# mvenouziou/Boosted_DETR

Measured on AMD Instinct MI355X. Metric: images/sec training step (fwd+matcher+loss+bwd), 640x640 N=100, higher is better.
Workload: dtype f32 (conv/GEMM products as 3 split-f16 [fwd] / split-bf16 [grad] MFMA products, f32 accumulate)

## Files before the change

boosted_detr_amd/_lib.py:

```python
from __future__ import annotations

import ctypes as C
import os
from pathlib import Path

_LIB_PATH = Path(os.environ.get("BDETR_LIB") or Path(__file__).resolve().parent / "csrc" / "libbdetr.so")
_lib = None

c_f32p = C.c_void_p
c_i32p = C.c_void_p
c_i64p = C.c_void_p
c_stream = C.c_void_p


class ConvDesc(C.Structure):
    _fields_ = [(n, C.c_int) for n in ("N", "H", "W", "C", "K", "R", "S", "stride", "pad", "OH", "OW")]


class GemmDesc(C.Structure):
    _fields_ = [
        ("I", C.c_int), ("J", C.c_int), ("R", C.c_int), ("nb0", C.c_int), ("nb1", C.c_int),
        ("a", C.c_void_p), ("lda", C.c_int64), ("sa0", C.c_int64), ("sa1", C.c_int64), ("a_rcontig", C.c_int),
        ("b", C.c_void_p), ("ldb", C.c_int64), ("sb0", C.c_int64), ("sb1", C.c_int64), ("b_rcontig", C.c_int),
        ("c", C.c_void_p), ("ldc", C.c_int64), ("sc0", C.c_int64), ("sc1", C.c_int64),
        ("bias", C.c_void_p), ("alpha", C.c_float), ("act", C.c_int), ("accumulate", C.c_int), ("splitk", C.c_int),
        ("grad", C.c_int),
    ]


class BnAffine(C.Structure):
    _fields_ = [("mean", C.c_void_p), ("rstd", C.c_void_p), ("gamma", C.c_void_p), ("beta", C.c_void_p)]


class BnBwdFuse(C.Structure):
    _fields_ = [("y", C.c_void_p), ("mean", C.c_void_p), ("rstd", C.c_void_p), ("gamma", C.c_void_p), ("beta", C.c_void_p), ("relu", C.c_int),
                ("part_g", C.c_void_p), ("part_gx", C.c_void_p), ("relu_mask", C.c_void_p),
                ("y2", C.c_void_p), ("mean2", C.c_void_p), ("rstd2", C.c_void_p), ("part_gx2", C.c_void_p)]


class RowchainFwdDesc(C.Structure):
    _fields_ = ([("M", C.c_int64), ("nstages", C.c_int), ("eps", C.c_float), ("rate", C.c_float), ("ctx", C.c_void_p), ("resid", C.c_void_p),
                 ("w", C.c_void_p * 3), ("bias", C.c_void_p * 3)]
                + [(n, C.c_void_p) for n in ("g1", "b1", "g2", "b2", "pre1", "x1", "mean1", "rstd1", "h", "pre2", "x2", "mean2", "rstd2")]
                + [("seed1", C.c_uint64), ("seed2", C.c_uint64), ("seed_base", C.c_void_p)])


class RowchainBwdDesc(C.Structure):
    _fields_ = ([("M", C.c_int64), ("nstages", C.c_int), ("rate", C.c_float)]
                + [(n, C.c_void_p) for n in ("dout", "pre2", "mean2", "rstd2", "g2", "h", "pre1", "mean1", "rstd1", "g1")]
                + [("wt", C.c_void_p * 3)]
                + [(n, C.c_void_p) for n in ("G2", "G1", "G0", "dresid", "dctx", "partials")]
                + [("seed1", C.c_uint64), ("seed2", C.c_uint64), ("seed_base", C.c_void_p)])
# ... 27 lines not shown
    "bdetr_prof_dump": (I, [C.c_char_p]),
    "bdetr_image_prep": (I, [P, I, I, I, P, I, I, P]),
    "bdetr_tokens_prepare": (I, [P, P, L, I, I, I, P, P, P]),
    "bdetr_augment_ws_floats": (I, [I]),
    "bdetr_augment": (I, [P, P, P, P, I, I, I, P, P]),
    "bdetr_jpeg_quality_ws_bytes": (C.c_int64, [I, I, I]),
    "bdetr_jpeg_quality": (I, [P, P, P, I, I, I, P, P]),
    "bdetr_augment_jpeg": (I, [P, P, P, P, P, I, I, I, P, P, P]),
    "bdetr_conv2d_fwd": (I, [P, P, P, P, C.POINTER(ConvDesc), I, P, P, P]),
    "bdetr_conv2d_fwd_stat_chunks": (I, [C.POINTER(ConvDesc)]),
    "bdetr_conv2d_bwd_data": (I, [P, P, P, C.POINTER(ConvDesc), I, P]),
    "bdetr_conv2d_bwd_weight": (I, [P, P, P, C.POINTER(ConvDesc), I, P]),
    "bdetr_conv2d_bwd_weight_splitk": (I, [C.POINTER(ConvDesc)]),
    "bdetr_bn_apply_p16": (I, [P, P, P, P, P, P, I, C.POINTER(BnAffine), I, P, P, P, P, P, L, I, P]),
    "bdetr_bn_bwd_p16": (I, [P, P, I, P, P, P, P, P, I, I, P, P, P, P, P, P, P, P, I, L, I, P]),
    "bdetr_bn_bwd_p16_even_pixels": (I, [P, P, I, P, P, P, P, P, I, I, P, P, P, P, P, P, I, I, I, I, I, P]),
    "bdetr_p16_supported": (I, [C.POINTER(ConvDesc)]),
    "bdetr_p16_pack": (I, [P, L, P, P, P, P]),
    "bdetr_p16_unpack": (I, [P, I, L, P, P]),
    "bdetr_p16_pack_conv_weights": (I, [P, I, I, I, I, P, P, P, P]),
    "bdetr_p16_pack_conv_weights_multi": (I, [P, I, P, P]),
    "bdetr_p16_conv2d_fwd_stat_chunks": (I, [C.POINTER(ConvDesc)]),
    "bdetr_p16_conv2d_fwd": (I, [P, P, P, P, C.POINTER(ConvDesc), I, P, P, P]),
    "bdetr_p16_conv2d_bwd_data": (I, [P, P, P, C.POINTER(ConvDesc), I, P]),
    "bdetr_p16_conv2d_bwd_data_stat_chunks": (I, [C.POINTER(ConvDesc)]),
    "bdetr_p16_conv2d_bwd_data_masked_accum": (I, [P, P, P, P, C.POINTER(ConvDesc), C.POINTER(BnBwdFuse), P]),
    "bdetr_p16_conv2d_bwd_data_masked_accum_compact": (I, [P, P, P, P, P, C.POINTER(ConvDesc), C.POINTER(BnBwdFuse), P]),
    "bdetr_relu_mask_apply": (I, [P, P, C.c_int64, P]),
    "bdetr_p16_conv2d_bwd_data_bnstats": (I, [P, P, P, C.POINTER(ConvDesc), C.POINTER(BnBwdFuse), P]),
    "bdetr_p16_conv2d_bwd_weight_splitk": (I, [C.POINTER(ConvDesc)]),
    "bdetr_p16_conv2d_bwd_weight": (I, [P, P, P, C.POINTER(ConvDesc), I, P]),
    "bdetr_p16_conv2d_bwd_weight_xf16": (I, [P, P, P, C.POINTER(ConvDesc), I, P]),
    "bdetr_gemm": (I, [C.POINTER(GemmDesc), P]),
    "bdetr_gemm_ws": (I, [C.POINTER(GemmDesc), P, L, P]),
    "bdetr_splitk_workspace_elems": (L, [L, L, I]),
    "bdetr_conv2d_bwd_weight_ws": (I, [P, P, P, C.POINTER(ConvDesc), I, P, L, P]),
    "bdetr_p16_conv2d_bwd_weight_ws": (I, [P, I, P, P, C.POINTER(ConvDesc), I, P, L, P]),
    "bdetr_gemm_grouped": (I, [C.POINTER(GemmDesc), I, P]),
    "bdetr_colsum_chunks": (I, [L]),
    "bdetr_colsum": (I, [P, L, I, P, P, P]),
# ... 107 lines not shown
```

boosted_detr_amd/csrc/gemm_common.h:

```cpp
#pragma once
#include "common.h"
#include <type_traits>

namespace bdgemm {

enum { ST_STORE = 0, ST_ACCUM = 1, ST_ATOMIC = 2 };
enum { AR_FP32 = 0, AR_BF16X3 = 1, AR_FP16X3 = 2, AR_P16_F16 = 3, AR_P16_BF16 = 4, AR_BF16X6 = 5 };

struct GemmParams {
    int I, J, R;
    int nb1;
    int splitk, r_chunk;
    int tiles_i, tiles_j;
    float* c; int64_t ldc, sc0, sc1;
    const float* bias; float alpha; int act; int mode;
    float* stat_sum; float* stat_sq;
    int vec_store;
    int rowmap;
    int rm_OW, rm_OHOW, rm_H, rm_W, rm_stride;
    int rm_off;
    int ngroups;
    const float* ga[4]; const float* gb[4]; float* gc[4]; const float* gbias[4]; int gI[4];
    const float* bnb_y; const float* bnb_mean; const float* bnb_rstd; const float* bnb_gamma; const float* bnb_beta;
    int bnb_relu; float* bnb_sum_g; float* bnb_sum_gx;
    const unsigned long long* bnb_mask;
    const float* bnb2_y; const float* bnb2_mean; const float* bnb2_rstd; float* bnb2_sum_gx;
    const unsigned long long* acc_mask;
    const float* acc_src; int acc_H, acc_W;
    int b_f16;
#ifdef BDETR_SGEMM_DIAG
    int dbg;
#endif
};

#ifdef BDETR_SGEMM_DIAG
#define BDETR_DBG(g, bits) (((g).dbg & (bits)) != 0)
#else
#define BDETR_DBG(g, bits) false
#endif

inline void init_params(GemmParams& g) {
// ... 174 lines not shown
                            if constexpr (MASKED) on = ((bbits[k] >> e) & 1u) != 0u;
                            else on = !g.bnb_relu || (__builtin_fmaf(yv[k][e] - bnv[0][e], bnv[1][e] * bnv[2][e], bnv[3][e]) > 0.f);
                            const float ge = on ? val[k][e] : 0.f;
                            bnv[4][e] += ge; bnv[5][e] += ge * ((yv[k][e] - bnv[0][e]) * bnv[1][e]);
                            if constexpr (BNB2) bn2[2][e] += ge * ((y2v[k][e] - bn2[0][e]) * bn2[1][e]);
                        }
                    }
                }
            }
            if constexpr (BNB) {
                static_assert(NT * 8 <= LDS_FLOATS, "reduction scratch must fit");
                __syncthreads();
                *reinterpret_cast<f32x4*>(lds + tid * 8) = bnv[4];
                *reinterpret_cast<f32x4*>(lds + tid * 8 + 4) = bnv[5];
                __syncthreads();
                if (tid < V_PER_ROW && jok) {
                    f32x4 a = {0, 0, 0, 0}, b = a;
#pragma unroll
                    for (int k = 0; k < RSTEP; ++k) {
                        a += *reinterpret_cast<const f32x4*>(lds + (tid + k * V_PER_ROW) * 8);
                        b += *reinterpret_cast<const f32x4*>(lds + (tid + k * V_PER_ROW) * 8 + 4);
                    }
                    *reinterpret_cast<f32x4*>(g.bnb_sum_g + (int64_t)tile_i * g.J + jc) = a;
                    *reinterpret_cast<f32x4*>(g.bnb_sum_gx + (int64_t)tile_i * g.J + jc) = b;
                }
                if constexpr (BNB2) {
                    __syncthreads();
                    *reinterpret_cast<f32x4*>(lds + tid * 4) = bn2[2];
                    __syncthreads();
                    if (tid < V_PER_ROW && jok) {
                        f32x4 c = {0, 0, 0, 0};
#pragma unroll
                        for (int k = 0; k < RSTEP; ++k) c += *reinterpret_cast<const f32x4*>(lds + (tid + k * V_PER_ROW) * 4);
                        *reinterpret_cast<f32x4*>(g.bnb2_sum_gx + (int64_t)tile_i * g.J + jc) = c;
                    }
                }
            }
        };
        using T = std::true_type; using F = std::false_type;
        const bool accum = g.mode == ST_ACCUM;
        if constexpr (BNB2_ONLY) { vec_out(F{}, T{}, T{}, T{}, T{}, F{}); return; }
        if constexpr (COMPACT_ONLY) {
            if (g.bnb_y != nullptr) vec_out(F{}, T{}, T{}, T{}, F{}, T{});
            else vec_out(F{}, T{}, F{}, T{}, F{}, T{});
            return;
// ... 59 lines not shown
```

boosted_detr_amd/csrc/norm.hip:

```cpp
#include "common.h"
#include "p16.h"

namespace {

struct ColGeom { int tx, ty, gx; };
inline ColGeom col_geom(int C) {
    int c4 = C / 4;
    int tx = 1; while (tx < c4 && tx < 64) tx <<= 1;
    ColGeom g; g.tx = tx; g.ty = 256 / tx; g.gx = (c4 + tx - 1) / tx; return g;
}

template <class F>
__global__ __launch_bounds__(256) void colreduce2_kernel(F f, int64_t rows, int C, int tx, int64_t rows_per_chunk,
                                                         float* __restrict__ pa, float* __restrict__ pb) {
    __shared__ f32x4 sa[256], sb[256];
    const int tid = threadIdx.x;
    const int cx = tid % tx, ry = tid / tx, ty = 256 / tx;
    const int c = (blockIdx.x * tx + cx) * 4;
    const int64_t r0 = (int64_t)blockIdx.y * rows_per_chunk;
    const int64_t r1 = min(rows, r0 + rows_per_chunk);
    f32x4 a = {0, 0, 0, 0}, b = {0, 0, 0, 0};
    if (c < C) {
        int64_t r = r0 + ry;
        for (; r + ty < r1; r += 2 * ty) {
// ... 89 lines not shown
                                                            float* oa, float* ob) {
    __shared__ double s1[256], s2[256];
    const int cx = threadIdx.x & 7, py = threadIdx.x >> 3;
    const int c = blockIdx.x * 8 + cx;
    double a = 0, b = 0;
    if (c < C) {
        int p = py;
        for (; p + 7 * 32 < nparts; p += 8 * 32) {
            float va[8], vb[8];
#pragma unroll
            for (int u = 0; u < 8; ++u) { va[u] = pa[(int64_t)(p + 32 * u) * C + c]; vb[u] = pb[(int64_t)(p + 32 * u) * C + c]; }
#pragma unroll
            for (int u = 0; u < 8; ++u) { a += va[u]; b += vb[u]; }
        }
        for (; p < nparts; p += 32) { a += pa[(int64_t)p * C + c]; b += pb[(int64_t)p * C + c]; }
    }
    s1[threadIdx.x] = a; s2[threadIdx.x] = b;
    __syncthreads();
    for (int s = 16; s > 0; s >>= 1) {
        if (py < s) { s1[threadIdx.x] += s1[threadIdx.x + 8 * s]; s2[threadIdx.x] += s2[threadIdx.x + 8 * s]; }
        __syncthreads();
    }
    if (py == 0 && c < C) { oa[c] = (float)s1[cx]; ob[c] = (float)s2[cx]; }
}

struct BnFinalizeArgs { int64_t rows; float eps, momentum; int bessel; float* mean; float* rstd; float* mmean; float* mvar; int* guard; };

template <bool FINALIZE>
__global__ __launch_bounds__(256) void reduce_partials2_kernel(const float* __restrict__ pa, const float* __restrict__ pb, int nparts, int C,
                                                               float* __restrict__ oa, float* __restrict__ ob, BnFinalizeArgs fin) {
// ... 780 lines not shown
    }
}
}

extern "C" int bdetr_relu_mask_apply(float* x, const uint64_t* relu_mask, int64_t n, void* stream) {
    BDETR_CHECK_ARG(x && relu_mask && n > 0 && n % 4 == 0, "bdetr_relu_mask_apply: bad arguments (n %% 4 == 0 required)");
    hipLaunchKernelGGL(relu_mask_apply_kernel, dim3(ew_grid(n / 4, 256, 2)), dim3(256), 0, (hipStream_t)stream, x,
                       reinterpret_cast<const unsigned long long*>(relu_mask), n / 4);
    return bdetr_launch_status("relu_mask_apply");
}

static int bn_bwd_p16_impl(const float* dout, const void* out, int out_p16, const float* x, const float* mean,
                           const float* rstd, const float* gamma, const float* beta, int relu, int frozen,
                           float* dx32, void* dx_bf16, float* dgamma, float* dbeta, float* dresidual,
                           float* ws, const float* pre_g, const float* pre_gx, int pre_n, int64_t rows, int C, int even_h, int even_w, void* stream,
                           int dout_compact = 0) {
    BDETR_CHECK_ARG(!dout_compact || (even_h > 0 && even_h % 2 == 0 && even_w % 2 == 0 && pre_g == nullptr && dresidual == nullptr),
                    "bdetr_bn_bwd_p16_even_pixels: a compact dout needs an even map, the even-pixel reduction and no residual-gradient output");
    BDETR_CHECK_ARG(!dout_compact || rows * C / 4 < ((int64_t)1 << 32), "bdetr_bn_bwd_p16_even_pixels: compact dout: more than 2^32 float4s");
    BDETR_CHECK_ARG(dout && x && mean && rstd && gamma && dx_bf16 && dgamma && dbeta && (ws || pre_g) && rows > 0 && C > 0 && C % 8 == 0,
                    "bdetr_bn_bwd_p16: bad arguments (C %% 8 == 0 required)");
    BDETR_CHECK_ARG((pre_g == nullptr) == (pre_gx == nullptr) && (pre_g == nullptr || pre_n > 0), "bdetr_bn_bwd_p16: pre_g / pre_gx / pre_n inconsistent");
    BDETR_CHECK_ARG(!relu || out || beta, "bdetr_bn_bwd_p16: relu needs the forward output, or beta to recompute the mask from x");
    hipStream_t st = (hipStream_t)stream;
    ColGeom g = col_geom(C);
    int64_t rpc = chunk_rows_for(rows, chunks_for_width(g.gx), 64);
    int nch = (int)cdiv64(rows, rpc);
    float* pa = ws; float* pb = ws + (int64_t)nch * C;
    if (pre_g != nullptr) {
        sum_partials2(pre_g, pre_gx, pre_n, C, dbeta, dgamma, st);
    } else {
        BnBwdFn f{dout, reinterpret_cast<const float*>(out), x, mean, rstd, gamma, beta, C, relu, out_p16, even_h, even_w, dout_compact};
        int64_t red_rows = rows;
        if (even_h > 0) {
            red_rows = rows / ((int64_t)even_h * even_w) * ((even_h + 1) / 2) * ((even_w + 1) / 2);
            rpc = chunk_rows_for(red_rows, chunks_for_width(g.gx), 64);
            nch = (int)cdiv64(red_rows, rpc);
            pb = ws + (int64_t)nch * C;
        }
        hipLaunchKernelGGL((colreduce2_kernel<BnBwdFn>), dim3(g.gx, nch), dim3(256), 0, st, f, red_rows, C, g.tx, rpc, pa, pb);
        sum_partials2(pa, pb, nch, C, dbeta, dgamma, st);
    }
    const int64_t n4 = rows * C / 4;
    hipLaunchKernelGGL(bn_bwd_apply_p16_kernel, dim3(channel_aligned_grid(n4, C)), dim3(256), 0, st, dout, out, out_p16, x, mean, rstd, gamma, beta, dgamma, dbeta,
                       relu, frozen, dx32, dx_bf16, dresidual, n4, C / 4, 1.0f / (float)rows, dout_compact ? even_h : 0, dout_compact ? even_w : 0);
    return bdetr_launch_status("bn_bwd_p16");
}

extern "C" int bdetr_bn_bwd_p16(const float* dout, const void* out, int out_p16, const float* x, const float* mean,
                                const float* rstd, const float* gamma, const float* beta, int relu, int frozen,
                                float* dx32, void* dx_bf16, float* dgamma, float* dbeta, float* dresidual,
                                float* ws, const float* pre_g, const float* pre_gx, int pre_n, int64_t rows, int C, void* stream) {
    return bn_bwd_p16_impl(dout, out, out_p16, x, mean, rstd, gamma, beta, relu, frozen, dx32, dx_bf16, dgamma, dbeta, dresidual, ws, pre_g, pre_gx, pre_n,
                           rows, C, 0, 0, stream);
}

extern "C" int bdetr_bn_bwd_p16_even_pixels(const float* dout, const void* out, int out_p16, const float* x, const float* mean,
                                            const float* rstd, const float* gamma, const float* beta, int relu, int frozen,
                                            float* dx32, void* dx_bf16, float* dgamma, float* dbeta, float* dresidual,
                                            float* ws, int N, int H, int W, int C, int dout_compact, void* stream) {
    BDETR_CHECK_ARG(N > 0 && H > 0 && W > 0 && ws && (int64_t)N * H * W < (int64_t)1 << 31, "bdetr_bn_bwd_p16_even_pixels: bad geometry");
    return bn_bwd_p16_impl(dout, out, out_p16, x, mean, rstd, gamma, beta, relu, frozen, dx32, dx_bf16, dgamma, dbeta, dresidual, ws, nullptr, nullptr, 0,
                           (int64_t)N * H * W, C, H, W, stream, dout_compact);
}

extern "C" int bdetr_add_dropout_layernorm_fwd(const float* x, const float* y, const float* gamma, const float* beta,
                                               float* out, float* mean, float* rstd, int64_t rows, int D,
                                               float eps, float rate, uint64_t seed, const uint64_t* seed_base, void* stream) {
    BDETR_CHECK_ARG(x && y && gamma && beta && out && mean && rstd && rows > 0, "bdetr_add_dropout_layernorm_fwd: null/empty argument");
// ... 55 lines not shown
```

boosted_detr_amd/csrc/sgemm.hip:

```cpp
#include "gemm_common.h"
#include "p16.h"
#include <stdlib.h>
#include <string.h>
#include <type_traits>
#include <utility>

using namespace bdgemm;

namespace {

constexpr int BK = 32;
constexpr unsigned OOB = 0xFFFFFFF0u;
constexpr unsigned NUM_RECORDS = 0xFFFFFF00u;

typedef __bf16 bf16x8 __attribute__((ext_vector_type(8)));
typedef _Float16 f16x8 __attribute__((ext_vector_type(8)));
typedef unsigned int u32x4 __attribute__((ext_vector_type(4)));
typedef unsigned int u32x2 __attribute__((ext_vector_type(2)));
typedef short s16x4 __attribute__((ext_vector_type(4)));
typedef __attribute__((address_space(3))) void lds_void;

__device__ __forceinline__ __amdgpu_buffer_rsrc_t make_rsrc(const void* p, unsigned records = NUM_RECORDS) {
    const unsigned long long a = reinterpret_cast<unsigned long long>(p);
    const unsigned lo = __builtin_amdgcn_readfirstlane((unsigned)a), hi = __builtin_amdgcn_readfirstlane((unsigned)(a >> 32));
// ... 783 lines not shown
}

static int bwd_data_hconv(const bdetr_conv_desc* d) {
    if (!(d->R == 3 && d->S == 3 && d->stride == 1 && d->pad == 1)) return 0;
    return hconv_tile((int64_t)d->N * d->H * d->W, d->W, d->K, d->C, false);
}

extern "C" int bdetr_p16_conv2d_bwd_data_stat_chunks(const bdetr_conv_desc* d) {
    if (check_conv(d, "bdetr_p16_conv2d_bwd_data_stat_chunks")) return -1;
    const bool dense = d->R == 1 && d->S == 1 && d->pad == 0;
    if (const int ht = bwd_data_hconv(d)) return (int)cdiv64((int64_t)d->N * d->H * d->W, ht / 1000);
    const int t = (dense && d->stride == 1) ? dense_vec_tile(d) : bwd_data_tile(d);
    return (int)cdiv64(dense ? (int64_t)d->N * d->OH * d->OW : (int64_t)d->N * d->H * d->W, TILE_BM[t]);
}

static int p16_bwd_data(const void* dy_bf16, const void* wt_bf16, float* dx, const bdetr_conv_desc* d, int accumulate,
                        const bdetr_bn_bwd_fuse* bn, const uint64_t* acc_mask, void* stream, const float* acc_src = nullptr) {
    if (int e = check_conv(d, "bdetr_p16_conv2d_bwd_data")) return e;
    BDETR_CHECK_ARG(dy_bf16 && wt_bf16 && dx, "bdetr_p16_conv2d_bwd_data: null pointer");
    hipStream_t st = (hipStream_t)stream;
    const int M = d->N * d->OH * d->OW;
    GemmParams g; init_params(g);
    g.c = dx; g.ldc = d->C; g.mode = accumulate ? ST_ACCUM : ST_STORE;
    g.acc_mask = reinterpret_cast<const unsigned long long*>(acc_mask);
    g.acc_src = acc_src; g.acc_H = d->H; g.acc_W = d->W;
    if (bn != nullptr) {
        const bool dense11 = d->R == 1 && d->S == 1 && d->pad == 0 && d->stride == 1;
        BDETR_CHECK_ARG((!accumulate || dense11) && d->stride == 1 && d->C % 4 == 0 && aligned16(dx) && aligned16(bn->y),
                        "bdetr_p16_conv2d_bwd_data_bnstats: needs 16-byte aligned rows, stride 1, and a plain store unless the conv is 1x1");
        BDETR_CHECK_ARG(bn->relu_mask == nullptr || dense11, "bdetr_p16_conv2d_bwd_data_bnstats: a bit-mask ReLU decision needs a 1x1 stride-1 conv");
        BDETR_CHECK_ARG(bn->y && bn->mean && bn->rstd && bn->gamma && bn->beta && bn->part_g && bn->part_gx, "bdetr_p16_conv2d_bwd_data_bnstats: null pointer");
        g.bnb_y = bn->y; g.bnb_mean = bn->mean; g.bnb_rstd = bn->rstd; g.bnb_gamma = bn->gamma; g.bnb_beta = bn->beta;
        g.bnb_relu = bn->relu; g.bnb_sum_g = bn->part_g; g.bnb_sum_gx = bn->part_gx;
        g.bnb_mask = reinterpret_cast<const unsigned long long*>(bn->relu_mask);
        if (bn->y2 != nullptr) {
            BDETR_CHECK_ARG(acc_mask != nullptr && bn->relu_mask != nullptr && bn->mean2 && bn->rstd2 && bn->part_gx2 && aligned16(bn->y2),
                            "bdetr_p16_conv2d_bwd_data_masked_accum: the second BatchNorm's sums ride a masked accumulate with masked sums");
            g.bnb2_y = bn->y2; g.bnb2_mean = bn->mean2; g.bnb2_rstd = bn->rstd2; g.bnb2_sum_gx = bn->part_gx2;
        }
    }
    if (d->R == 1 && d->S == 1 && d->pad == 0) {
        g.I = M; g.J = d->C; g.R = d->K;
        if (d->stride > 1) {
            if (!accumulate) {
                if (int e = bdetr_zero_bytes(dx, sizeof(float) * (size_t)d->N * d->H * d->W * d->C, st)) return e;
            }
            g.rowmap = 1; g.rm_OW = d->OW; g.rm_OHOW = d->OH * d->OW; g.rm_H = d->H; g.rm_W = d->W; g.rm_stride = d->stride;
        }
        PDense a{dy_bf16, (unsigned)d->K, M, d->K};
        PDense b{wt_bf16, (unsigned)d->K, d->C, d->K};
        const bool vec = !g.rowmap && (g.mode == ST_ACCUM || g.bnb_y != nullptr);
        return launch_any<RRDense, RRDense, false, false>(a, b, g, 1, st, 0, vec ? dense_vec_tile(d) : bwd_data_tile(d));
    }
    BDETR_CHECK_ARG(d->stride == 1 && d->R == d->S, "bdetr_p16_conv2d_bwd_data: stride>1 only for 1x1 convs; square kernels only");
// ... 162 lines not shown
```

boosted_detr_amd/engine.py:

```python
from __future__ import annotations

import math
import zlib
from typing import Callable, Dict, List, Optional, Sequence

import numpy as np
import torch

from . import kernels as K

_DEVICE = None


def device() -> torch.device:
    global _DEVICE
    if _DEVICE is None:
        if not torch.cuda.is_available():
            raise RuntimeError("boosted_detr_amd needs an AMD GPU (HIP device); there is no CPU execution path")
        _DEVICE = torch.device("cuda", torch.cuda.current_device())
    return _DEVICE


def to_device(a, dtype=torch.float32) -> torch.Tensor:
    if isinstance(a, torch.Tensor):
# ... 145 lines not shown
    r = getattr(g, "_grad_info", None)
    if r is None:
        r = g._grad_info = GradInfo()
    return r


def own(t: torch.Tensor) -> torch.Tensor:
    tag(t).owned = True
    return t


def dense_contribution(g: torch.Tensor, keep_even=None) -> None:
    r = info(g)
    if r is _NO_INFO:
        return
    r.bnb_parts = r.bnb_parts_shortcut = None
    if r.even_pixels != keep_even:
        r.even_pixels = None


def materialise(g):
    r = info(g)
    if r.compact_even is not None:
        N, H, W = r.compact_even
        d = torch.empty(N, H, W, g.shape[-1], dtype=g.dtype, device=g.device)
        K.zero_(d)
        d[:, ::2, ::2] = g.view(N, H // 2, W // 2, g.shape[-1])
        mask, r = r.lazy_mask, tag(d)
        r.owned, r.even_pixels, r.lazy_mask = True, (N, H, W), mask
        g = d
# ... 522 lines not shown
```

boosted_detr_amd/kernels.py:

```python
from __future__ import annotations

import ctypes as C
from dataclasses import dataclass
from typing import Optional, Tuple

import numpy as np
import torch

from . import _lib
from ._lib import BnAffine, BnBwdFuse, ConvDesc, GemmDesc, LossDesc, RowchainBwdDesc, RowchainFwdDesc, check

ACT_NONE, ACT_RELU, ACT_TANH = 0, 1, 2


_LAUNCH_STREAM = [None]


def set_launch_stream(handle: Optional[int]) -> Optional[int]:
    prev = _LAUNCH_STREAM[0]
    _LAUNCH_STREAM[0] = handle
    return prev


GEMM_FP32, GEMM_BF16X3, GEMM_MIXED, GEMM_SPLIT, GEMM_BF16X6 = 0, 1, 2, 3, 4
# ... 19 lines not shown


import os as _os

_DETERMINISTIC = [_os.environ.get("BDETR_DETERMINISTIC", "0") == "1"]


def set_deterministic(on: bool) -> bool:
    prev = _DETERMINISTIC[0]
    _DETERMINISTIC[0] = bool(on)
    return prev


def deterministic() -> bool:
    return _DETERMINISTIC[0]


def _splitk_ws(rows: int, cols: int, sk: int, like: torch.Tensor):
    if not _DETERMINISTIC[0] or sk <= 1:
        return None, 0
    n = int(_lib.lib().bdetr_splitk_workspace_elems(rows, cols, sk))
    return torch.empty(n, dtype=torch.float32, device=like.device), n


class gemm_precision:

    def __init__(self, mode):
        self.mode = mode

    def __enter__(self):
# ... 246 lines not shown
    rows, Cc = x2d.shape
    dxb = torch.empty_like(x2d)
    dx32 = torch.empty_like(x2d) if want_fp32 else None
    dgamma = empty(Cc, like=x2d) if dgamma is None else dgamma
    dbeta = empty(Cc, like=x2d) if dbeta is None else dbeta
    dres = torch.empty_like(x2d) if want_residual_grad else None
    ws = empty(2 * Cc * L.bdetr_bn_bwd_chunks(rows), like=x2d) if pre is None else None
    if even_pixels is not None and pre is None:
        N, H, W = even_pixels
        assert N * H * W == rows
        assert not dout_compact or (dres is None and dout.numel() == N * (H // 2) * (W // 2) * Cc and H % 2 == 0 and W % 2 == 0)
        check(L.bdetr_bn_bwd_p16_even_pixels(_p(dout), _p(out), int(out_p16), _p(x2d), _p(mean), _p(rstd), _p(gamma), _p(beta), int(relu), int(frozen),
                                             _p(dx32), _p(dxb), _p(dgamma), _p(dbeta), _p(dres), _p(ws), N, H, W, Cc, int(dout_compact), _stream()), "bn_bwd_p16_even_pixels")
        return dxb, dx32, dgamma, dbeta, dres
    assert not dout_compact, "a compact dout goes through the even-pixel reduction (even_pixels=(N, H, W), no pre)"
    pg, pgx, pn = pre if pre is not None else (None, None, 0)
    check(L.bdetr_bn_bwd_p16(_p(dout), _p(out), int(out_p16), _p(x2d), _p(mean), _p(rstd), _p(gamma), _p(beta), int(relu), int(frozen), _p(dx32),
                             _p(dxb), _p(dgamma), _p(dbeta), _p(dres), _p(ws), _p(pg), _p(pgx), int(pn), rows, Cc, _stream()), "bn_bwd_p16")
    return dxb, dx32, dgamma, dbeta, dres


def p16_pack_conv_weights_multi(table: torch.Tensor) -> None:
    _chk(table, dtype=torch.int64)
    check(_lib.lib().bdetr_p16_pack_conv_weights_multi(_p(table), table.shape[0], _p(overflow_flag()), _stream()), "p16_pack_conv_weights_multi")


def p16_conv2d_fwd(x_f16, w_f16, bias, g: ConvGeom, act: int = ACT_NONE, want_stats: bool = False):
    _chk(x_f16, w_f16, bias)
    L = _lib.lib()
    d = g.desc()
    y = empty(g.N, g.OH, g.OW, g.K, like=x_f16)
# ... 12 lines not shown
def p16_conv2d_bwd_data(dy_bf16, wt_bf16, g: ConvGeom, dx: Optional[torch.Tensor] = None, accumulate: bool = False):
    _chk(dy_bf16, wt_bf16, dx)
    d = g.desc()
    if dx is None:
        assert not accumulate
        dx = empty(g.N, g.H, g.W, g.C, like=dy_bf16)
    check(_lib.lib().bdetr_p16_conv2d_bwd_data(_p(dy_bf16), _p(wt_bf16), _p(dx), C.byref(d), int(accumulate), _stream()), "p16_conv2d_bwd_data")
    return dx


def relu_mask_apply_(x: torch.Tensor, relu_mask: torch.Tensor) -> torch.Tensor:
    _chk(x)
    _chk(relu_mask, dtype=torch.int64)
    check(_lib.lib().bdetr_relu_mask_apply(_p(x), _p(relu_mask), x.numel(), _stream()), "relu_mask_apply")
    return x


def p16_conv2d_bwd_data_masked_accum(dy_bf16, wt_bf16, g: ConvGeom, dx: torch.Tensor, relu_mask: torch.Tensor, bn_ctx=None, bn_ctx2=None, old_even=None):
    _chk(dy_bf16, wt_bf16, dx)
    _chk(relu_mask, dtype=torch.int64)
    L = _lib.lib()
    d = g.desc()
    if old_even is not None:
        _chk(old_even)
        assert bn_ctx2 is None and old_even.numel() * 4 == dx.numel() and g.H % 2 == 0 and g.W % 2 == 0

        def launch(fuse):
            check(L.bdetr_p16_conv2d_bwd_data_masked_accum_compact(_p(dy_bf16), _p(wt_bf16), _p(dx), _p(old_even), _p(relu_mask), C.byref(d), fuse, _stream()),
                  "p16_conv2d_bwd_data_masked_accum_compact")
    else:
        def launch(fuse):
            check(L.bdetr_p16_conv2d_bwd_data_masked_accum(_p(dy_bf16), _p(wt_bf16), _p(dx), _p(relu_mask), C.byref(d), fuse, _stream()),
                  "p16_conv2d_bwd_data_masked_accum")
    if bn_ctx is None:
        launch(None)
        return dx
    y_prev, mean, rstd, gamma, beta, bits_prev = bn_ctx
    _chk(y_prev, mean, rstd, gamma, beta)
    _chk(bits_prev, dtype=torch.int64)
    n = L.bdetr_p16_conv2d_bwd_data_stat_chunks(C.byref(d))
    if n <= 0:
        check(-1, "p16_conv2d_bwd_data_stat_chunks")
    pg, pgx = empty(n, g.C, like=dy_bf16), empty(n, g.C, like=dy_bf16)
    f = BnBwdFuse(_p(y_prev), _p(mean), _p(rstd), _p(gamma), _p(beta), 1, _p(pg), _p(pgx), _p(bits_prev))
    pgx2 = None
    if bn_ctx2 is not None:
        y0, mean0, rstd0 = bn_ctx2
        _chk(y0, mean0, rstd0)
        pgx2 = empty(n, g.C, like=dy_bf16)
        f.y2, f.mean2, f.rstd2, f.part_gx2 = _p(y0), _p(mean0), _p(rstd0), _p(pgx2)
    launch(C.byref(f))
    if pgx2 is not None:
        return dx, (pg, pgx, n), (pg, pgx2, n)
    return dx, (pg, pgx, n)


def p16_conv2d_bwd_data_bnstats(dy_bf16, wt_bf16, g: ConvGeom, y_prev, mean, rstd, gamma, beta, relu: bool):
    _chk(dy_bf16, wt_bf16, y_prev, mean, rstd, gamma, beta)
    L = _lib.lib()
    d = g.desc()
    dx = empty(g.N, g.H, g.W, g.C, like=dy_bf16)
    n = L.bdetr_p16_conv2d_bwd_data_stat_chunks(C.byref(d))
    if n <= 0:
        check(-1, "p16_conv2d_bwd_data_stat_chunks")
    pg, pgx = empty(n, g.C, like=dy_bf16), empty(n, g.C, like=dy_bf16)
    f = BnBwdFuse(_p(y_prev), _p(mean), _p(rstd), _p(gamma), _p(beta), int(relu), _p(pg), _p(pgx), None)
    check(L.bdetr_p16_conv2d_bwd_data_bnstats(_p(dy_bf16), _p(wt_bf16), _p(dx), C.byref(d), C.byref(f), _stream()), "p16_conv2d_bwd_data_bnstats")
    return dx, (pg, pgx, n)


def p16_conv2d_bwd_weight(x_bf16, dy_bf16, g: ConvGeom, dw: Optional[torch.Tensor] = None, prezeroed: bool = False, x_f16: bool = False):
    _chk(x_bf16, dy_bf16, dw)
    L = _lib.lib()
    d = g.desc()
    if dw is None:
        dw = empty(g.K, g.R, g.S, g.C, like=x_bf16)
        prezeroed = False
    sk = L.bdetr_p16_conv2d_bwd_weight_splitk(C.byref(d))
    if sk > 1 and not prezeroed:
        check(L.bdetr_zero(_p(dw), dw.numel(), _stream()), "zero")
    ws, n = _splitk_ws(g.K, g.R * g.S * g.C, sk, x_bf16)
    check(L.bdetr_p16_conv2d_bwd_weight_ws(_p(x_bf16), int(x_f16), _p(dy_bf16), _p(dw), C.byref(d), sk, _p(ws), n, _stream()), "p16_conv2d_bwd_weight")
    return dw
# ... 625 lines not shown
```

boosted_detr_amd/ops.py:

```python
from __future__ import annotations

import math
import os
import weakref
from typing import Optional

import numpy as np
import torch

from . import kernels as K
from . import _lib
from .engine import WEIGHTS_VERSION, Variable, current_tape, dense_contribution, info, materialise, own, side_task, tag

_dropout_site = [0]
_dropout_seed_dev = [None]


def dropout_seed_tensor() -> torch.Tensor:
    if _dropout_seed_dev[0] is None:
        _dropout_seed_dev[0] = torch.full((1,), 0x5EED, dtype=torch.int64, device="cuda")
    return _dropout_seed_dev[0]


def set_dropout_seed(seed: int, write: bool = True) -> None:
# ... 330 lines not shown
    if lazy_bits is not None:
        mask_src, mode, bn_relu = lazy_bits, 2, True
    even = gi.even_pixels if (EVEN_PIXELS and gi.even_pixels == omap) else None
    if compact is not None:
        assert lazy_skip and pre is None, "a compact even-pixel gradient is handed on to the skip merge as it is"
        even = compact
    dyb, _, _, _, dres = K.bn_bwd_p16(g2d, mask_src, y2d, mean, rstd, bn.gamma.value, bn_relu, False, want_residual_grad=want_res and not lazy_skip,
                                      dgamma=sg.buf, dbeta=sb.buf, beta=bn.beta.value, out_p16=mode, pre=pre, even_pixels=even,
                                      dout_compact=compact is not None)
    if lazy_skip:
        dres = own(g_out.view(res_shape) if compact is None else g_out)
        ri = tag(dres)
        ri.lazy_mask = relu_bits
        if gi.bnb_parts_shortcut is not None and res_bn is not None:
            ri.bnb_parts = gi.bnb_parts_shortcut
    elif want_res:
        dres = own(dres.view(res_shape))
    sg.commit()
    sb.commit()
    return dyb, (dres if want_res else None)


def _p16_input_grad(dyb4, w: Variable, g, xa: ActInfo, acc):
    N, H, W, Cin = g.N, g.H, g.W, g.C
    imap = (N, H, W)
    one = g.R == 1 and g.S == 1 and g.pad == 0
    s1, s2 = one and g.stride == 1, one and g.stride == 2
    s2c = s2 and COMPACT_S2 and H % 2 == 0 and W % 2 == 0
    gc = K.ConvGeom(N, g.OH, g.OW, Cin, g.K, 1, 1, 1, 0) if s2c else None
    keep_even = imap if s2 else None
    _, wt = _PACKED.get(w)
# ... 406 lines not shown
```

boosted_detr_amd/training.py:

```python
from __future__ import annotations

import contextlib
import glob
import math
import os
import sys
import time
from dataclasses import dataclass
from typing import Dict, Iterable, List, NamedTuple, Optional

import numpy as np
import torch

from . import _lib
from . import engine
from . import kernels as K
from . import ops
from .engine import Layer, Tape, Variable, bump_weights_version, device, join_side_stream, recording, to_device


class CosineDecayRestarts:

    def __init__(self, initial_learning_rate, first_decay_steps, t_mul=2.0, m_mul=1.0, alpha=0.0):
        self.initial_learning_rate = float(initial_learning_rate)
# ... 896 lines not shown
            ops.set_dropout_seed(self._step_seed())
            self.optimizer.stage_lr()
            keep = (self.steps_done, self.optimizer.iterations)
            if self._dp is not None:
                self._dp.drain()
            cap = engine.SegmentedCapture()
            engine.set_capture(cap)
            prev_launch = K.set_launch_stream(None)
            try:
                cap.begin_main()
                logs = self._device_step(static, stage_scalars=False)
                cap.end_main()
                cap.sides.append(None)
            except BaseException:
                cap.abort()
                self.steps_done, self.optimizer.iterations = keep
                raise
            finally:
                engine.set_capture(None)
                K.set_launch_stream(prev_launch)
            cap.done = []
            if cap.CENSUS:
                self._graph_census = cap.census()
            self.steps_done, self.optimizer.iterations = keep
            entry = (cap, static, logs, (list(self._step_losses), list(self._loss_roots), dict(self._step_metrics)))
            self._graphs[sig] = entry
        cap, static, logs, book = entry
        for k, v in data.items():
            if v is not static[k]:
                static[k].copy_(v)
# ... 228 lines not shown
```

include/bdetr.h:

```cpp
#ifndef BDETR_H
#define BDETR_H
#include <stdint.h>
#ifdef __cplusplus
extern "C" {
#endif

#define BDETR_ABI_VERSION 8

int         bdetr_abi_version(void);
const char* bdetr_last_error(void);
int         bdetr_device_cus(void);

int         bdetr_low_priority_stream_create(void** stream_out);
int         bdetr_stream_priority_range(int* least, int* greatest);
int         bdetr_side_stream_candidates(void* main_stream, int ncand, int loads, int ticks, void** streams_out, float* scores_ms, float* unloaded_ms);
int         bdetr_stream_destroy(void* stream);

enum { BDETR_GEMM_FP32 = 0, BDETR_GEMM_BF16X3 = 1, BDETR_GEMM_MIXED = 2, BDETR_GEMM_SPLIT = 3, BDETR_GEMM_BF16X6 = 4 };
int         bdetr_set_gemm_precision(int mode);
int         bdetr_get_gemm_precision(void);

int bdetr_prof_enable(int on);
int bdetr_prof_read(double* total_ms, int64_t* launches, double* flops);
int bdetr_prof_read_arith(int arith, double* total_ms, int64_t* launches, double* flops);
// ... 30 lines not shown
                            const bdetr_conv_desc* d, int splitk, void* stream);
int bdetr_conv2d_bwd_weight_splitk(const bdetr_conv_desc* d);
int bdetr_conv2d_bwd_weight_ws(const float* x, const float* dy, float* dw,
                               const bdetr_conv_desc* d, int splitk, float* ws, int64_t ws_elems, void* stream);
int64_t bdetr_splitk_workspace_elems(int64_t I, int64_t J, int splitk);

typedef struct { const float* mean; const float* rstd; const float* gamma; const float* beta; } bdetr_bn_affine;
int bdetr_bn_apply_p16(const float* x, const float* mean, const float* rstd, const float* gamma,
                       const float* beta, const void* residual, int residual_p16, const bdetr_bn_affine* residual_bn, int relu, float* out32,
                       void* out_f16, void* out_bf16, uint64_t* relu_mask, int* overflow_flag, int64_t rows, int C,
                       void* stream);
int bdetr_bn_bwd_p16(const float* dout, const void* out, int out_p16, const float* x, const float* mean,
                     const float* rstd, const float* gamma, const float* beta, int relu, int frozen,
                     float* dx32, void* dx_bf16, float* dgamma, float* dbeta, float* dresidual,
                     float* ws, const float* pre_g, const float* pre_gx, int pre_n, int64_t rows, int C, void* stream);
int bdetr_bn_bwd_p16_even_pixels(const float* dout, const void* out, int out_p16, const float* x, const float* mean,
                                 const float* rstd, const float* gamma, const float* beta, int relu, int frozen,
                                 float* dx32, void* dx_bf16, float* dgamma, float* dbeta, float* dresidual,
                                 float* ws, int N, int H, int W, int C,
                                 int dout_compact , void* stream);
int bdetr_p16_supported(const bdetr_conv_desc* d);
int bdetr_p16_pack(const float* x, int64_t n, void* f16_out, void* bf16_out, int* overflow_flag, void* stream);
int bdetr_p16_unpack(const void* p, int is_f16, int64_t n, float* out, void* stream);
int bdetr_p16_pack_conv_weights(const float* w, int K, int R, int S, int C, void* w_f16, void* wt_bf16,
                                int* overflow_flag, void* stream);
int bdetr_p16_pack_conv_weights_multi(const int64_t* table, int ntensors, int* overflow_flag, void* stream);
int bdetr_p16_conv2d_fwd_stat_chunks(const bdetr_conv_desc* d);
int bdetr_p16_conv2d_fwd(const void* x_f16, const void* w_f16, const float* bias, float* y,
                         const bdetr_conv_desc* d, int act, float* stat_sum, float* stat_sq, void* stream);
int bdetr_p16_conv2d_bwd_data(const void* dy_bf16, const void* wt_bf16, float* dx,
                              const bdetr_conv_desc* d, int accumulate, void* stream);
typedef struct {
    const float* y; const float* mean; const float* rstd; const float* gamma; const float* beta; int relu;
    float* part_g; float* part_gx;
    const uint64_t* relu_mask;
    const float* y2; const float* mean2; const float* rstd2; float* part_gx2;
} bdetr_bn_bwd_fuse;
int bdetr_p16_conv2d_bwd_data_stat_chunks(const bdetr_conv_desc* d);
int bdetr_relu_mask_apply(float* x, const uint64_t* relu_mask, int64_t n, void* stream);
int bdetr_p16_conv2d_bwd_data_masked_accum(const void* dy_bf16, const void* wt_bf16, float* dx, const uint64_t* relu_mask,
                                           const bdetr_conv_desc* d, const bdetr_bn_bwd_fuse* bn , void* stream);
int bdetr_p16_conv2d_bwd_data_masked_accum_compact(const void* dy_bf16, const void* wt_bf16, float* dx, const float* old_even,
                                                   const uint64_t* relu_mask, const bdetr_conv_desc* d, const bdetr_bn_bwd_fuse* bn, void* stream);
int bdetr_p16_conv2d_bwd_data_bnstats(const void* dy_bf16, const void* wt_bf16, float* dx,
                                      const bdetr_conv_desc* d, const bdetr_bn_bwd_fuse* bn, void* stream);
int bdetr_p16_conv2d_bwd_weight_splitk(const bdetr_conv_desc* d);
int bdetr_p16_conv2d_bwd_weight(const void* x_bf16, const void* dy_bf16, float* dw,
                                const bdetr_conv_desc* d, int splitk, void* stream);
int bdetr_p16_conv2d_bwd_weight_xf16(const void* x_f16, const void* dy_bf16, float* dw,
                                     const bdetr_conv_desc* d, int splitk, void* stream);
int bdetr_p16_conv2d_bwd_weight_ws(const void* x, int x_is_f16, const void* dy_bf16, float* dw,
                                   const bdetr_conv_desc* d, int splitk, float* ws, int64_t ws_elems, void* stream);

// ... 179 lines not shown
```

Baseline: 641.5.

## Accumulate fused BN-backward partial sums into atomic slot tables instead of per-tile partials

In the 1x1 backward-data GEMM epilogue that fuses BatchNorm-backward statistics, each tile now atomically adds its column sums into a small fixed table of slots (tile index mod slots) instead of writing one partial row per tile. A new reduction kernel sums the slot rows into dgamma/dbeta and zeroes the table for reuse, so the follow-up reduction reads far fewer rows and needs no per-call partial buffers. The cost is atomic contention and non-deterministic summation order, so the path is turned off in deterministic mode. It also adds persistent per-layer tables that have to be cleared when partials are dropped or a capture aborts.

New measurement: 645.7, median of 6. Within noise of the previous version (+0.7%).

```diff
diff --git a/boosted_detr_amd/_lib.py b/boosted_detr_amd/_lib.py
--- a/boosted_detr_amd/_lib.py
+++ b/boosted_detr_amd/_lib.py
@@ -35,7 +35,8 @@
 class BnBwdFuse(C.Structure):
     _fields_ = [("y", C.c_void_p), ("mean", C.c_void_p), ("rstd", C.c_void_p), ("gamma", C.c_void_p), ("beta", C.c_void_p), ("relu", C.c_int),
                 ("part_g", C.c_void_p), ("part_gx", C.c_void_p), ("relu_mask", C.c_void_p),
-                ("y2", C.c_void_p), ("mean2", C.c_void_p), ("rstd2", C.c_void_p), ("part_gx2", C.c_void_p)]
+                ("y2", C.c_void_p), ("mean2", C.c_void_p), ("rstd2", C.c_void_p), ("part_gx2", C.c_void_p),
+                ("slots", C.c_int), ("part_g2", C.c_void_p)]
 
 
 class RowchainFwdDesc(C.Structure):
@@ -93,6 +94,7 @@
     "bdetr_conv2d_bwd_weight_splitk": (I, [C.POINTER(ConvDesc)]),
     "bdetr_bn_apply_p16": (I, [P, P, P, P, P, P, I, C.POINTER(BnAffine), I, P, P, P, P, P, L, I, P]),
     "bdetr_bn_bwd_p16": (I, [P, P, I, P, P, P, P, P, I, I, P, P, P, P, P, P, P, P, I, L, I, P]),
+    "bdetr_bn_bwd_p16_slots": (I, [P, P, I, P, P, P, P, P, I, I, P, P, P, P, P, P, P, I, L, I, P]),
     "bdetr_bn_bwd_p16_even_pixels": (I, [P, P, I, P, P, P, P, P, I, I, P, P, P, P, P, P, I, I, I, I, I, P]),
     "bdetr_p16_supported": (I, [C.POINTER(ConvDesc)]),
     "bdetr_p16_pack": (I, [P, L, P, P, P, P]),
@@ -103,6 +105,7 @@
     "bdetr_p16_conv2d_fwd": (I, [P, P, P, P, C.POINTER(ConvDesc), I, P, P, P]),
     "bdetr_p16_conv2d_bwd_data": (I, [P, P, P, C.POINTER(ConvDesc), I, P]),
     "bdetr_p16_conv2d_bwd_data_stat_chunks": (I, [C.POINTER(ConvDesc)]),
+    "bdetr_p16_conv2d_bwd_data_stat_slots": (I, [C.POINTER(ConvDesc), I]),
     "bdetr_p16_conv2d_bwd_data_masked_accum": (I, [P, P, P, P, C.POINTER(ConvDesc), C.POINTER(BnBwdFuse), P]),
     "bdetr_p16_conv2d_bwd_data_masked_accum_compact": (I, [P, P, P, P, P, C.POINTER(ConvDesc), C.POINTER(BnBwdFuse), P]),
     "bdetr_relu_mask_apply": (I, [P, P, C.c_int64, P]),
diff --git a/boosted_detr_amd/csrc/gemm_common.h b/boosted_detr_amd/csrc/gemm_common.h
--- a/boosted_detr_amd/csrc/gemm_common.h
+++ b/boosted_detr_amd/csrc/gemm_common.h
@@ -25,6 +25,7 @@
     int bnb_relu; float* bnb_sum_g; float* bnb_sum_gx;
     const unsigned long long* bnb_mask;
     const float* bnb2_y; const float* bnb2_mean; const float* bnb2_rstd; float* bnb2_sum_gx;
+    int bnb_slots; float* bnb2_sum_g;
     const unsigned long long* acc_mask;
     const float* acc_src; int acc_H, acc_W;
     int b_f16;
@@ -229,7 +230,21 @@
                 *reinterpret_cast<f32x4*>(lds + tid * 8) = bnv[4];
                 *reinterpret_cast<f32x4*>(lds + tid * 8 + 4) = bnv[5];
                 __syncthreads();
-                if (tid < V_PER_ROW && jok) {
+                float slot_g = 0.f;
+                const int slot_row = g.bnb_slots > 0 ? tile_i % g.bnb_slots : 0;
+                if (g.bnb_slots > 0) {
+                    if constexpr (2 * BN <= NT) {
+                        if (tid < 2 * BN) {
+                            const int q = tid >= BN ? 1 : 0, col = tid - q * BN;
+                            const float* src = lds + (col >> 2) * 8 + q * 4 + (col & 3);
+                            float sum = 0.f;
+#pragma unroll
+                            for (int k = 0; k < RSTEP; ++k) sum += src[k * V_PER_ROW * 8];
+                            if (j0 + col < g.J) unsafeAtomicAdd((q ? g.bnb_sum_gx : g.bnb_sum_g) + (int64_t)slot_row * g.J + j0 + col, sum);
+                            if (q == 0) slot_g = sum;
+                        }
+                    }
+                } else if (tid < V_PER_ROW && jok) {
                     f32x4 a = {0, 0, 0, 0}, b = a;
 #pragma unroll
                     for (int k = 0; k < RSTEP; ++k) {
@@ -243,7 +258,20 @@
                     __syncthreads();
                     *reinterpret_cast<f32x4*>(lds + tid * 4) = bn2[2];
                     __syncthreads();
-                    if (tid < V_PER_ROW && jok) {
+                    if (g.bnb_slots > 0) {
+                        if constexpr (2 * BN <= NT) {
+                            if (tid < BN) {
+                                const float* src = lds + (tid >> 2) * 4 + (tid & 3);
+                                float sum = 0.f;
+#pragma unroll
+                                for (int k = 0; k < RSTEP; ++k) sum += src[k * V_PER_ROW * 4];
+                                if (j0 + tid < g.J) {
+                                    unsafeAtomicAdd(g.bnb2_sum_gx + (int64_t)slot_row * g.J + j0 + tid, sum);
+                                    unsafeAtomicAdd(g.bnb2_sum_g + (int64_t)slot_row * g.J + j0 + tid, slot_g);
+                                }
+                            }
+                        }
+                    } else if (tid < V_PER_ROW && jok) {
                         f32x4 c = {0, 0, 0, 0};
 #pragma unroll
                         for (int k = 0; k < RSTEP; ++k) c += *reinterpret_cast<const f32x4*>(lds + (tid + k * V_PER_ROW) * 4);
diff --git a/boosted_detr_amd/csrc/norm.hip b/boosted_detr_amd/csrc/norm.hip
--- a/boosted_detr_amd/csrc/norm.hip
+++ b/boosted_detr_amd/csrc/norm.hip
@@ -127,6 +127,35 @@
             for (int u = 0; u < 8; ++u) { a += va[u]; b += vb[u]; }
         }
         for (; p < nparts; p += 32) { a += pa[(int64_t)p * C + c]; b += pb[(int64_t)p * C + c]; }
+    }
+    s1[threadIdx.x] = a; s2[threadIdx.x] = b;
+    __syncthreads();
+    for (int s = 16; s > 0; s >>= 1) {
+        if (py < s) { s1[threadIdx.x] += s1[threadIdx.x + 8 * s]; s2[threadIdx.x] += s2[threadIdx.x + 8 * s]; }
+        __syncthreads();
+    }
+    if (py == 0 && c < C) { oa[c] = (float)s1[cx]; ob[c] = (float)s2[cx]; }
+}
+
+__global__ __launch_bounds__(256) void sum_slots2_kernel(float* __restrict__ pa, float* __restrict__ pb, int S, int C, float* oa, float* ob) {
+    __shared__ double s1[256], s2[256];
+    const int cx = threadIdx.x & 7, py = threadIdx.x >> 3;
+    const int c = blockIdx.x * 8 + cx;
+    double a = 0, b = 0;
+    if (c < C) {
+        float va[8], vb[8];
+#pragma unroll
+        for (int u = 0; u < 8; ++u) {
+            const int p = py + 32 * u;
+            va[u] = vb[u] = 0.f;
+            if (p < S) { va[u] = pa[(int64_t)p * C + c]; vb[u] = pb[(int64_t)p * C + c]; }
+        }
+#pragma unroll
+        for (int u = 0; u < 8; ++u) {
+            const int p = py + 32 * u;
+            a += va[u]; b += vb[u];
+            if (p < S) { pa[(int64_t)p * C + c] = 0.f; pb[(int64_t)p * C + c] = 0.f; }
+        }
     }
     s1[threadIdx.x] = a; s2[threadIdx.x] = b;
     __syncthreads();
@@ -937,7 +966,7 @@
                            const float* rstd, const float* gamma, const float* beta, int relu, int frozen,
                            float* dx32, void* dx_bf16, float* dgamma, float* dbeta, float* dresidual,
                            float* ws, const float* pre_g, const float* pre_gx, int pre_n, int64_t rows, int C, int even_h, int even_w, void* stream,
-                           int dout_compact = 0) {
+                           int dout_compact = 0, bool pre_slots = false) {
     BDETR_CHECK_ARG(!dout_compact || (even_h > 0 && even_h % 2 == 0 && even_w % 2 == 0 && pre_g == nullptr && dresidual == nullptr),
                     "bdetr_bn_bwd_p16_even_pixels: a compact dout needs an even map, the even-pixel reduction and no residual-gradient output");
     BDETR_CHECK_ARG(!dout_compact || rows * C / 4 < ((int64_t)1 << 32), "bdetr_bn_bwd_p16_even_pixels: compact dout: more than 2^32 float4s");
@@ -950,7 +979,9 @@
     int64_t rpc = chunk_rows_for(rows, chunks_for_width(g.gx), 64);
     int nch = (int)cdiv64(rows, rpc);
     float* pa = ws; float* pb = ws + (int64_t)nch * C;
-    if (pre_g != nullptr) {
+    if (pre_slots) {
+        hipLaunchKernelGGL(sum_slots2_kernel, dim3((C + 7) / 8), dim3(256), 0, st, const_cast<float*>(pre_g), const_cast<float*>(pre_gx), pre_n, C, dbeta, dgamma);
+    } else if (pre_g != nullptr) {
         sum_partials2(pre_g, pre_gx, pre_n, C, dbeta, dgamma, st);
     } else {
         BnBwdFn f{dout, reinterpret_cast<const float*>(out), x, mean, rstd, gamma, beta, C, relu, out_p16, even_h, even_w, dout_compact};
@@ -976,6 +1007,15 @@
                                 float* ws, const float* pre_g, const float* pre_gx, int pre_n, int64_t rows, int C, void* stream) {
     return bn_bwd_p16_impl(dout, out, out_p16, x, mean, rstd, gamma, beta, relu, frozen, dx32, dx_bf16, dgamma, dbeta, dresidual, ws, pre_g, pre_gx, pre_n,
                            rows, C, 0, 0, stream);
+}
+
+extern "C" int bdetr_bn_bwd_p16_slots(const float* dout, const void* out, int out_p16, const float* x, const float* mean,
+                                      const float* rstd, const float* gamma, const float* beta, int relu, int frozen,
+                                      float* dx32, void* dx_bf16, float* dgamma, float* dbeta, float* dresidual,
+                                      float* slot_g, float* slot_gx, int slots, int64_t rows, int C, void* stream) {
+    BDETR_CHECK_ARG(slot_g && slot_gx && slot_g != slot_gx && slots > 0 && slots <= 256, "bdetr_bn_bwd_p16_slots: two tables of 1 .. 256 rows required");
+    return bn_bwd_p16_impl(dout, out, out_p16, x, mean, rstd, gamma, beta, relu, frozen, dx32, dx_bf16, dgamma, dbeta, dresidual, nullptr, slot_g, slot_gx, slots,
+                           rows, C, 0, 0, stream, 0, true);
 }
 
 extern "C" int bdetr_bn_bwd_p16_even_pixels(const float* dout, const void* out, int out_p16, const float* x, const float* mean,
diff --git a/boosted_detr_amd/csrc/sgemm.hip b/boosted_detr_amd/csrc/sgemm.hip
--- a/boosted_detr_amd/csrc/sgemm.hip
+++ b/boosted_detr_amd/csrc/sgemm.hip
@@ -821,6 +821,14 @@
     return (int)cdiv64(dense ? (int64_t)d->N * d->OH * d->OW : (int64_t)d->N * d->H * d->W, TILE_BM[t]);
 }
 
+extern "C" int bdetr_p16_conv2d_bwd_data_stat_slots(const bdetr_conv_desc* d, int want) {
+    if (check_conv(d, "bdetr_p16_conv2d_bwd_data_stat_slots")) return -1;
+    BDETR_CHECK_ARG(want >= 0 && want <= 256, "bdetr_p16_conv2d_bwd_data_stat_slots: 0 .. 256 slots");
+    if (want == 0 || !(d->R == 1 && d->S == 1 && d->pad == 0 && d->stride == 1)) return 0;
+    const int64_t tiles_i = cdiv64((int64_t)d->N * d->OH * d->OW, TILE_BM[dense_vec_tile(d)]);
+    return tiles_i > 4 * (int64_t)want ? want : 0;
+}
+
 static int p16_bwd_data(const void* dy_bf16, const void* wt_bf16, float* dx, const bdetr_conv_desc* d, int accumulate,
                         const bdetr_bn_bwd_fuse* bn, const uint64_t* acc_mask, void* stream, const float* acc_src = nullptr) {
     if (int e = check_conv(d, "bdetr_p16_conv2d_bwd_data")) return e;
@@ -845,6 +853,11 @@
                             "bdetr_p16_conv2d_bwd_data_masked_accum: the second BatchNorm's sums ride a masked accumulate with masked sums");
             g.bnb2_y = bn->y2; g.bnb2_mean = bn->mean2; g.bnb2_rstd = bn->rstd2; g.bnb2_sum_gx = bn->part_gx2;
         }
+        if (bn->slots != 0) {
+            BDETR_CHECK_ARG(bn->slots > 0 && bn->slots == bdetr_p16_conv2d_bwd_data_stat_slots(d, bn->slots) && (bn->y2 == nullptr || bn->part_g2 != nullptr),
+                            "bdetr_p16_conv2d_bwd_data_bnstats: slots must be what bdetr_p16_conv2d_bwd_data_stat_slots returns (and part_g2 set with y2)");
+            g.bnb_slots = bn->slots; g.bnb2_sum_g = bn->part_g2;
+        }
     }
     if (d->R == 1 && d->S == 1 && d->pad == 0) {
         g.I = M; g.J = d->C; g.R = d->K;
diff --git a/boosted_detr_amd/engine.py b/boosted_detr_amd/engine.py
--- a/boosted_detr_amd/engine.py
+++ b/boosted_detr_amd/engine.py
@@ -183,6 +183,9 @@
     r = info(g)
     if r is _NO_INFO:
         return
+    if r.bnb_parts is not None or r.bnb_parts_shortcut is not None:
+        K.bn_slot_parts_drop(r.bnb_parts)
+        K.bn_slot_parts_drop(r.bnb_parts_shortcut)
     r.bnb_parts = r.bnb_parts_shortcut = None
     if r.even_pixels != keep_even:
         r.even_pixels = None
diff --git a/boosted_detr_amd/kernels.py b/boosted_detr_amd/kernels.py
--- a/boosted_detr_amd/kernels.py
+++ b/boosted_detr_amd/kernels.py
@@ -57,6 +57,33 @@
 
 def deterministic() -> bool:
     return _DETERMINISTIC[0]
+
+
+_BN_SLOT_TABLES = {}
+
+
+def bn_sum_slots() -> int:
+    return 0 if _DETERMINISTIC[0] else int(_os.environ.get("BDETR_BN_SUM_SLOTS", "64"))
+
+
+def _bn_slot_tables(gamma: torch.Tensor, slots: int, cols: int) -> torch.Tensor:
+    key = (gamma.device.index, gamma.data_ptr(), slots, cols)
+    t = _BN_SLOT_TABLES.get(key)
+    if t is None:
+        t = _BN_SLOT_TABLES[key] = torch.zeros(4, slots, cols, dtype=torch.float32, device=gamma.device)
+    return t
+
+
+def bn_slot_tables_zero() -> None:
+    for t in _BN_SLOT_TABLES.values():
+        with torch.cuda.device(t.device):
+            check(_lib.lib().bdetr_zero(_p(t), t.numel(), _stream()), "zero")
+
+
+def bn_slot_parts_drop(parts) -> None:
+    if parts is not None and len(parts) > 3:
+        for t in parts[:2]:
+            check(_lib.lib().bdetr_zero(_p(t), t.numel(), _stream()), "zero")
 
 
 def _splitk_ws(rows: int, cols: int, sk: int, like: torch.Tensor):
@@ -333,7 +360,11 @@
                                              _p(dx32), _p(dxb), _p(dgamma), _p(dbeta), _p(dres), _p(ws), N, H, W, Cc, int(dout_compact), _stream()), "bn_bwd_p16_even_pixels")
         return dxb, dx32, dgamma, dbeta, dres
     assert not dout_compact, "a compact dout goes through the even-pixel reduction (even_pixels=(N, H, W), no pre)"
-    pg, pgx, pn = pre if pre is not None else (None, None, 0)
+    pg, pgx, pn = pre[:3] if pre is not None else (None, None, 0)
+    if pre is not None and len(pre) > 3:
+        check(L.bdetr_bn_bwd_p16_slots(_p(dout), _p(out), int(out_p16), _p(x2d), _p(mean), _p(rstd), _p(gamma), _p(beta), int(relu), int(frozen), _p(dx32),
+                                       _p(dxb), _p(dgamma), _p(dbeta), _p(dres), _p(pg), _p(pgx), int(pn), rows, Cc, _stream()), "bn_bwd_p16_slots")
+        return dxb, dx32, dgamma, dbeta, dres
     check(L.bdetr_bn_bwd_p16(_p(dout), _p(out), int(out_p16), _p(x2d), _p(mean), _p(rstd), _p(gamma), _p(beta), int(relu), int(frozen), _p(dx32),
                              _p(dxb), _p(dgamma), _p(dbeta), _p(dres), _p(ws), _p(pg), _p(pgx), int(pn), rows, Cc, _stream()), "bn_bwd_p16")
     return dxb, dx32, dgamma, dbeta, dres
@@ -376,6 +407,16 @@
     _chk(relu_mask, dtype=torch.int64)
     check(_lib.lib().bdetr_relu_mask_apply(_p(x), _p(relu_mask), x.numel(), _stream()), "relu_mask_apply")
     return x
+
+
+def _bwd_data_stat_slots(d) -> int:
+    want = bn_sum_slots()
+    if want <= 0:
+        return 0
+    s = _lib.lib().bdetr_p16_conv2d_bwd_data_stat_slots(C.byref(d), want)
+    if s < 0:
+        check(-1, "p16_conv2d_bwd_data_stat_slots")
+    return s
 
 
 def p16_conv2d_bwd_data_masked_accum(dy_bf16, wt_bf16, g: ConvGeom, dx: torch.Tensor, relu_mask: torch.Tensor, bn_ctx=None, bn_ctx2=None, old_even=None):
@@ -403,18 +444,27 @@
     n = L.bdetr_p16_conv2d_bwd_data_stat_chunks(C.byref(d))
     if n <= 0:
         check(-1, "p16_conv2d_bwd_data_stat_chunks")
-    pg, pgx = empty(n, g.C, like=dy_bf16), empty(n, g.C, like=dy_bf16)
+    slots = _bwd_data_stat_slots(d)
+    if slots:
+        pg, pgx, pg2, pgx2s = _bn_slot_tables(gamma, slots, g.C).unbind(0)
+        n, mark = slots, (True,)
+    else:
+        pg, pgx = empty(n, g.C, like=dy_bf16), empty(n, g.C, like=dy_bf16)
+        mark = ()
     f = BnBwdFuse(_p(y_prev), _p(mean), _p(rstd), _p(gamma), _p(beta), 1, _p(pg), _p(pgx), _p(bits_prev))
+    f.slots = slots
     pgx2 = None
     if bn_ctx2 is not None:
         y0, mean0, rstd0 = bn_ctx2
         _chk(y0, mean0, rstd0)
-        pgx2 = empty(n, g.C, like=dy_bf16)
+        pgx2 = pgx2s if slots else empty(n, g.C, like=dy_bf16)
         f.y2, f.mean2, f.rstd2, f.part_gx2 = _p(y0), _p(mean0), _p(rstd0), _p(pgx2)
+        if slots:
+            f.part_g2 = _p(pg2)
     launch(C.byref(f))
     if pgx2 is not None:
-        return dx, (pg, pgx, n), (pg, pgx2, n)
-    return dx, (pg, pgx, n)
+        return dx, (pg, pgx, n) + mark, ((pg2 if slots else pg), pgx2, n) + mark
+    return dx, (pg, pgx, n) + mark
 
 
 def p16_conv2d_bwd_data_bnstats(dy_bf16, wt_bf16, g: ConvGeom, y_prev, mean, rstd, gamma, beta, relu: bool):
@@ -425,10 +475,17 @@
     n = L.bdetr_p16_conv2d_bwd_data_stat_chunks(C.byref(d))
     if n <= 0:
         check(-1, "p16_conv2d_bwd_data_stat_chunks")
-    pg, pgx = empty(n, g.C, like=dy_bf16), empty(n, g.C, like=dy_bf16)
+    slots = _bwd_data_stat_slots(d)
+    if slots:
+        pg, pgx = _bn_slot_tables(gamma, slots, g.C)[:2].unbind(0)
+        n, mark = slots, (True,)
+    else:
+        pg, pgx = empty(n, g.C, like=dy_bf16), empty(n, g.C, like=dy_bf16)
+        mark = ()
     f = BnBwdFuse(_p(y_prev), _p(mean), _p(rstd), _p(gamma), _p(beta), int(relu), _p(pg), _p(pgx), None)
+    f.slots = slots
     check(L.bdetr_p16_conv2d_bwd_data_bnstats(_p(dy_bf16), _p(wt_bf16), _p(dx), C.byref(d), C.byref(f), _stream()), "p16_conv2d_bwd_data_bnstats")
-    return dx, (pg, pgx, n)
+    return dx, (pg, pgx, n) + mark
 
 
 def p16_conv2d_bwd_weight(x_bf16, dy_bf16, g: ConvGeom, dw: Optional[torch.Tensor] = None, prezeroed: bool = False, x_f16: bool = False):
diff --git a/boosted_detr_amd/ops.py b/boosted_detr_amd/ops.py
--- a/boosted_detr_amd/ops.py
+++ b/boosted_detr_amd/ops.py
@@ -368,7 +368,10 @@
         ri.lazy_mask = relu_bits
         if gi.bnb_parts_shortcut is not None and res_bn is not None:
             ri.bnb_parts = gi.bnb_parts_shortcut
+        else:
+            K.bn_slot_parts_drop(gi.bnb_parts_shortcut)
     elif want_res:
+        K.bn_slot_parts_drop(gi.bnb_parts_shortcut)
         dres = own(dres.view(res_shape))
     sg.commit()
     sb.commit()
diff --git a/boosted_detr_amd/training.py b/boosted_detr_amd/training.py
--- a/boosted_detr_amd/training.py
+++ b/boosted_detr_amd/training.py
@@ -934,6 +934,7 @@
                 cap.sides.append(None)
             except BaseException:
                 cap.abort()
+                K.bn_slot_tables_zero()
                 self.steps_done, self.optimizer.iterations = keep
                 raise
             finally:
diff --git a/include/bdetr.h b/include/bdetr.h
--- a/include/bdetr.h
+++ b/include/bdetr.h
@@ -68,6 +68,10 @@
                      const float* rstd, const float* gamma, const float* beta, int relu, int frozen,
                      float* dx32, void* dx_bf16, float* dgamma, float* dbeta, float* dresidual,
                      float* ws, const float* pre_g, const float* pre_gx, int pre_n, int64_t rows, int C, void* stream);
+int bdetr_bn_bwd_p16_slots(const float* dout, const void* out, int out_p16, const float* x, const float* mean,
+                           const float* rstd, const float* gamma, const float* beta, int relu, int frozen,
+                           float* dx32, void* dx_bf16, float* dgamma, float* dbeta, float* dresidual,
+                           float* slot_g, float* slot_gx, int slots, int64_t rows, int C, void* stream);
 int bdetr_bn_bwd_p16_even_pixels(const float* dout, const void* out, int out_p16, const float* x, const float* mean,
                                  const float* rstd, const float* gamma, const float* beta, int relu, int frozen,
                                  float* dx32, void* dx_bf16, float* dgamma, float* dbeta, float* dresidual,
@@ -89,8 +93,10 @@
     float* part_g; float* part_gx;
     const uint64_t* relu_mask;
     const float* y2; const float* mean2; const float* rstd2; float* part_gx2;
+    int slots; float* part_g2;
 } bdetr_bn_bwd_fuse;
 int bdetr_p16_conv2d_bwd_data_stat_chunks(const bdetr_conv_desc* d);
+int bdetr_p16_conv2d_bwd_data_stat_slots(const bdetr_conv_desc* d, int want);
 int bdetr_relu_mask_apply(float* x, const uint64_t* relu_mask, int64_t n, void* stream);
 int bdetr_p16_conv2d_bwd_data_masked_accum(const void* dy_bf16, const void* wt_bf16, float* dx, const uint64_t* relu_mask,
                                            const bdetr_conv_desc* d, const bdetr_bn_bwd_fuse* bn , void* stream);
```
